# bao1029p/celestia-app

Measured on AMD Instinct MI355X. Metric: EDS+DAH squares/sec (128→256 sq, node) + RS GB/s & NMT SHA-256 hashes/sec, higher is better.
Workload: dtype u8; 1 GPU; 128x128 ODS -> 256x256 EDS + NMT row/col roots + DAH (configs[1]); k=128, global_batch=256, parallelism=squares sharded over 1 GPU(s), no collective, ods_layout=in place (Q0 of the EDS buffer)

## Files before the change

### celestia-app_amd/csrc/nmt.hip

```cpp
#include <hip/hip_runtime.h>
#include <stdint.h>
#include <stdlib.h>

#include "kernels.hpp"
#include "nmt_node.hpp"
#include "pipe_carve.hpp"
#include "sha256.hpp"

namespace dagpu {

constexpr int kLeafWave = 256;

__global__ __launch_bounds__(kLeafWave) void nmt_leaf_kernel(SquareArgs a, int row0, int nrows, int zero_status) {
  const int k = a.k;
  const long w = 2L * k;
  const long cells = w * w;
  const long span = nrows * w;
  const long total = span * a.nsq;
  const long gid = (long)blockIdx.x * kLeafWave + threadIdx.x;
  if (gid >= total) return;
  const long sq = gid / span;
  const long cell = row0 * w + (gid - sq * span);
  const long r = cell / w, c = cell - (cell / w) * w;
  const bool q0 = (r < k) && (c < k);
  if (zero_status && cell == 0) a.status[sq] = 0;
  const uint4* src = (const uint4*)(a.eds + sq * a.eds_sq_stride + cell * kShareSize);
  uint32_t st[8], ns[8];
  share_leaf_sha256(src, q0, st, ns);
  if (q0) {
    uint4* nsp = (uint4*)(a.ns_table + (sq * k * k + r * k + c) * 32);
    nsp[0] = make_uint4(ns[0], ns[1], ns[2], ns[3]);
    nsp[1] = make_uint4(ns[4], ns[5], ns[6], ns[7]);
  }
  uint4* out = (uint4*)(a.digests + (sq * cells + cell) * kDigest);
  out[0] = make_uint4(bswap32(st[0]), bswap32(st[1]), bswap32(st[2]), bswap32(st[3]));
  out[1] = make_uint4(bswap32(st[4]), bswap32(st[5]), bswap32(st[6]), bswap32(st[7]));
}

__device__ __forceinline__ void load_ns(const uint8_t* share, bool q0, uint32_t (&ns)[8]) {
  if (q0) {
    const uint4* p = (const uint4*)share;
    const uint4 v0 = p[0], v1 = p[1];
    ns[0] = v0.x; ns[1] = v0.y; ns[2] = v0.z; ns[3] = v0.w;
    ns[4] = v1.x; ns[5] = v1.y; ns[6] = v1.z; ns[7] = v1.w & 0xFFu;
  } else {
#pragma unroll
    for (int i = 0; i < 7; i++) ns[i] = 0xFFFFFFFFu;
    ns[7] = 0xFFu;
  }
}

constexpr uint32_t kParityRef = 0xFFFFFFFFu;

__device__ __forceinline__ void ns_by_ref(const uint8_t* ns_sq, uint32_t ref, uint32_t (&ns)[8]) {
  if (ref == kParityRef) {
#pragma unroll
    for (int i = 0; i < 7; i++) ns[i] = 0xFFFFFFFFu;
    ns[7] = 0xFFu;
  } else {
    const uint4* p = (const uint4*)(ns_sq + (long)ref * 32);
    const uint4 v0 = p[0], v1 = p[1];
    ns[0] = v0.x; ns[1] = v0.y; ns[2] = v0.z; ns[3] = v0.w;
    ns[4] = v1.x; ns[5] = v1.y; ns[6] = v1.z; ns[7] = v1.w;
  }
}

__device__ __forceinline__ void level_coords(long gid, int w, int per, long& sq, int& axis, int& idx, int& p) {
  const long blk = 2L * w * per;
  sq = gid / blk;
  const long g = gid - sq * blk;
  axis = g >= (long)w * per;
  const long g2 = g - (axis ? (long)w * per : 0);
  if (axis == 0) { idx = (int)(g2 / per); p = (int)(g2 - (long)idx * per); }
  else { p = (int)(g2 / w); idx = (int)(g2 - (long)p * w); }
}

__device__ __forceinline__ long level_rec(long sq, int w, int per, int axis, int idx, int p) {
  const long base = sq * 2L * w * per;
  return axis == 0 ? base + (long)idx * per + p : base + (long)w * per + (long)p * w + idx;
}

__global__ __launch_bounds__(256) void nmt_level1_kernel(SquareArgs a, uint8_t* out_rec, int final_level) {
  const int k = a.k;
  const int w = 2 * k;
  const int half = w / 2;
  const long gid = (long)blockIdx.x * 256 + threadIdx.x;
  const long total = a.nsq * 2L * w * half;
  if (gid >= total) return;
  long sq;
  int axis, idx, p;
  level_coords(gid, w, half, sq, axis, idx, p);
  const uint8_t* dig = a.digests + sq * (long)w * w * kDigest;
  const uint8_t* ns_sq = a.ns_table + sq * (long)k * k * 32;
  const int j0 = 2 * p, j1 = 2 * p + 1;
  const long cell0 = axis == 0 ? (long)idx * w + j0 : (long)j0 * w + idx;
  const long cell1 = axis == 0 ? (long)idx * w + j1 : (long)j1 * w + idx;
  const bool q00 = (idx < k) && (j0 < k), q01 = (idx < k) && (j1 < k);
  const uint32_t ref0 = q00 ? (axis == 0 ? (uint32_t)(idx * k + j0) : (uint32_t)(j0 * k + idx)) : kParityRef;
  const uint32_t ref1 = q01 ? (axis == 0 ? (uint32_t)(idx * k + j1) : (uint32_t)(j1 * k + idx)) : kParityRef;
  uint32_t nl[8], nr[8], dl[8], dr[8];
  ns_by_ref(ns_sq, ref0, nl);
  ns_by_ref(ns_sq, ref1, nr);
  load_digest(dig + cell0 * kDigest, dl);
  load_digest(dig + cell1 * kDigest, dr);
  if (q01) {
    bool bad = ns_less(nr, nl);
    if (j1 + 1 < k) {
      const uint32_t ref2 = axis == 0 ? (uint32_t)(idx * k + j1 + 1) : (uint32_t)((j1 + 1) * k + idx);
      uint32_t n2[8];
      ns_by_ref(ns_sq, ref2, n2);
      bad |= ns_less(n2, nr);
    }
    if (bad) atomicOr(&a.status[sq], kStatusPushOrder);
  }
  uint32_t st[8];
  const bool lpar = ns_is_parity(nl), rpar = ns_is_parity(nr);
  if (__all(lpar && rpar)) {
    auto get = [&](int P, int i) -> uint32_t {
      return P == 2 ? dl[i] : P == 5 ? dr[i] : 0xFFFFFFFFu;
    };
    sha_node_msg<true, true, true>(get, st);
  } else if (__all(lpar)) {
    auto get = [&](int P, int i) -> uint32_t {
      return P == 0 || P == 1 ? 0xFFFFFFFFu : P == 2 ? dl[i] : P == 3 || P == 4 ? nr[i] : dr[i];
    };
    sha_node_msg<true>(get, st);
  } else {
    auto get = [&](int P, int i) -> uint32_t {
      return P == 0 || P == 1 ? nl[i] : P == 2 ? dl[i] : P == 3 || P == 4 ? nr[i] : dr[i];
    };
    sha_node_msg(get, st);
  }
  uint32_t dg[8];
#pragma unroll
  for (int i = 0; i < 8; i++) dg[i] = bswap32(st[i]);
  if (final_level) {
    uint8_t* dst = (axis == 0 ? a.row_roots : a.col_roots) + (sq * w + idx) * kNodeSize;
    write_root(dst, nl, rpar ? nl : nr, dg);
  } else {
    const uint32_t lref = lpar ? kParityRef : ref0;
    const uint32_t rref = rpar ? kParityRef : ref1;
    uint4* o = (uint4*)(out_rec + gid * 48);
    o[0] = make_uint4(dg[0], dg[1], dg[2], dg[3]);
    o[1] = make_uint4(dg[4], dg[5], dg[6], dg[7]);
    o[2] = make_uint4(lref, rref == kParityRef ? lref : rref, 0u, 0u);
  }
}

__global__ __launch_bounds__(256) void nmt_level_kernel(SquareArgs a, const uint8_t* in_rec, uint8_t* out_rec,
                                                        int level, int final_level) {
  const int k = a.k;
  const int w = 2 * k;
  const int per = w >> level;
  const long gid = (long)blockIdx.x * 256 + threadIdx.x;
  const long total = a.nsq * 2L * w * per;
  if (gid >= total) return;
  long sq;
  int axis, idx, p;
  level_coords(gid, w, per, sq, axis, idx, p);
  const uint8_t* ns_sq = a.ns_table + sq * (long)k * k * 32;
  const uint4* li = (const uint4*)(in_rec + level_rec(sq, w, 2 * per, axis, idx, 2 * p) * 48);
  const uint4* ri = (const uint4*)(in_rec + level_rec(sq, w, 2 * per, axis, idx, 2 * p + 1) * 48);
  const uint4 l0 = li[0], l1 = li[1], l2 = li[2], r0 = ri[0], r1 = ri[1], r2 = ri[2];
  const uint32_t dl[8] = {l0.x, l0.y, l0.z, l0.w, l1.x, l1.y, l1.z, l1.w};
  const uint32_t dr[8] = {r0.x, r0.y, r0.z, r0.w, r1.x, r1.y, r1.z, r1.w};
  uint32_t lmn[8], lmx[8], rmn[8], rmx[8];
  ns_by_ref(ns_sq, l2.x, lmn);
  ns_by_ref(ns_sq, l2.y, lmx);
  ns_by_ref(ns_sq, r2.x, rmn);
  ns_by_ref(ns_sq, r2.y, rmx);
  uint32_t st[8];
  if (__all(l2.x == kParityRef && r2.x == kParityRef)) {
    auto get = [&](int P, int i) -> uint32_t {
      return P == 2 ? dl[i] : P == 5 ? dr[i] : 0xFFFFFFFFu;
    };
    sha_node_msg<true, true, true>(get, st);
  } else if (__all(l2.x == kParityRef)) {
    auto get = [&](int P, int i) -> uint32_t {
      return P <= 1 ? 0xFFFFFFFFu : P == 2 ? dl[i] : P == 3 ? rmn[i] : P == 4 ? rmx[i] : dr[i];
    };
    sha_node_msg<true>(get, st);
  } else {
    auto get = [&](int P, int i) -> uint32_t {
      return P == 0 ? lmn[i] : P == 1 ? lmx[i] : P == 2 ? dl[i] : P == 3 ? rmn[i] : P == 4 ? rmx[i] : dr[i];
    };
    sha_node_msg(get, st);
  }
  uint32_t dg[8];
#pragma unroll
  for (int i = 0; i < 8; i++) dg[i] = bswap32(st[i]);
  const bool rpar = r2.x == kParityRef;
  if (final_level) {
    uint8_t* dst = (axis == 0 ? a.row_roots : a.col_roots) + (sq * w + idx) * kNodeSize;
    if (rpar) write_root(dst, lmn, lmx, dg);
    else write_root(dst, lmn, rmx, dg);
  } else {
    uint4* o = (uint4*)(out_rec + gid * 48);
    o[0] = make_uint4(dg[0], dg[1], dg[2], dg[3]);
    o[1] = make_uint4(dg[4], dg[5], dg[6], dg[7]);
    o[2] = make_uint4(l2.x, rpar ? l2.y : r2.y, 0u, 0u);
  }
}

constexpr int kDahThreads = 1024;
constexpr int kDahChunk = 2048;

__device__ uint32_t* rfc_reduce(uint32_t* src, uint32_t* dst, int cur) {
  while (cur > 1) {
    const int next = cur / 2;
    for (int i = threadIdx.x; i < next; i += kDahThreads) {
      uint32_t m[32];
#pragma unroll
      for (int j = 0; j < 32; j++) m[j] = 0;
      uint32_t lft[8], rgt[8];
#pragma unroll
      for (int j = 0; j < 8; j++) { lft[j] = src[(2 * i) * 8 + j]; rgt[j] = src[(2 * i + 1) * 8 + j]; }
      m[0] = 0x01u;
      put_bytes<1>(m, lft);
      put_bytes<33>(m, rgt);
      m[65 >> 2] |= 0x80u << (8 * (65 & 3));
      uint32_t st[8];
      sha256_init(st);
#pragma unroll
      for (int blk = 0; blk < 2; blk++) {
        uint32_t wv[16];
#pragma unroll
        for (int j = 0; j < 16; j++) wv[j] = bswap32(m[16 * blk + j]);
        if (blk == 1) { wv[14] = 0; wv[15] = 65u * 8u; }
        sha256_compress(st, wv);
      }
#pragma unroll
      for (int j = 0; j < 8; j++) dst[i * 8 + j] = bswap32(st[j]);
    }
    __syncthreads();
    uint32_t* t = src;
    src = dst;
    dst = t;
    cur = next;
  }
  return src;
}

__device__ __forceinline__ void dah_leaf(const SquareArgs& a, long sq, int li, uint32_t* out) {
  const int w = 2 * a.k;
  const uint8_t* root = (li < w ? a.row_roots + (sq * w + li) * kNodeSize
                                : a.col_roots + (sq * w + (li - w)) * kNodeSize);
  uint32_t m[32];
#pragma unroll
  for (int j = 0; j < 32; j++) m[j] = 0;
  const uint16_t* r16 = (const uint16_t*)root;
#pragma unroll
  for (int h = 0; h < 45; h++) {
    const uint32_t v = r16[h];
    const int off = 1 + 2 * h;
    m[off >> 2] |= v << (8 * (off & 3));
    if ((off & 3) == 3) m[(off >> 2) + 1] |= v >> 8;
  }
  m[91 >> 2] |= 0x80u << (8 * (91 & 3));
  uint32_t st[8];
  sha256_init(st);
#pragma unroll
  for (int blk = 0; blk < 2; blk++) {
    uint32_t wv[16];
#pragma unroll
    for (int j = 0; j < 16; j++) wv[j] = bswap32(m[16 * blk + j]);
    if (blk == 1) { wv[14] = 0; wv[15] = 91u * 8u; }
    sha256_compress(st, wv);
  }
#pragma unroll
  for (int j = 0; j < 8; j++) out[j] = bswap32(st[j]);
}

__global__ __launch_bounds__(kDahThreads) void dah_kernel(SquareArgs a) {
  extern __shared__ __attribute__((aligned(16))) uint32_t lds[];
  const long sq = blockIdx.x;
  const int w = 2 * a.k;
  const int n = 2 * w;
  const int C = n < kDahChunk ? n : kDahChunk;
  uint32_t* sub = lds + (C + C / 2) * 8;
  for (int c0 = 0; c0 < n; c0 += C) {
    for (int i = threadIdx.x; i < C; i += kDahThreads) dah_leaf(a, sq, c0 + i, lds + i * 8);
    __syncthreads();
    const uint32_t* r = rfc_reduce(lds, lds + C * 8, C);
    if (threadIdx.x < 8) sub[(c0 / C) * 8 + threadIdx.x] = r[threadIdx.x];
    __syncthreads();
  }
  const uint32_t* root = rfc_reduce(sub, lds, n / C);
  if (threadIdx.x < 8) {
    uint32_t* out = (uint32_t*)(a.dah + sq * 32);
    out[threadIdx.x] = root[threadIdx.x];
  }
}

constexpr int kDahSub = 64;
__global__ __launch_bounds__(kDahSub) void dah_sub_kernel(SquareArgs a) {
  __shared__ __attribute__((aligned(16))) uint32_t buf[2][kDahSub * 8];
  const int n = 4 * a.k, per = n / kDahSub;
  const long sq = blockIdx.x / per;
  const int b = (int)(blockIdx.x % per);
  const int i = threadIdx.x;
  dah_leaf(a, sq, b * kDahSub + i, buf[0] + i * 8);
  int cur = kDahSub, src = 0;
  while (cur > 1) {
    __syncthreads();
    const int next = cur / 2;
    if (i < next) {
      uint32_t m[32];
#pragma unroll
      for (int j = 0; j < 32; j++) m[j] = 0;
      uint32_t lft[8], rgt[8];
#pragma unroll
      for (int j = 0; j < 8; j++) {
        lft[j] = buf[src][(2 * i) * 8 + j];
        rgt[j] = buf[src][(2 * i + 1) * 8 + j];
      }
      m[0] = 0x01u;
      put_bytes<1>(m, lft);
      put_bytes<33>(m, rgt);
      m[65 >> 2] |= 0x80u << (8 * (65 & 3));
      uint32_t st[8];
      sha256_init(st);
#pragma unroll
      for (int blk = 0; blk < 2; blk++) {
        uint32_t wv[16];
#pragma unroll
        for (int j = 0; j < 16; j++) wv[j] = bswap32(m[16 * blk + j]);
        if (blk == 1) { wv[14] = 0; wv[15] = 65u * 8u; }
        sha256_compress(st, wv);
      }
#pragma unroll
      for (int j = 0; j < 8; j++) buf[src ^ 1][i * 8 + j] = bswap32(st[j]);
    }
    src ^= 1;
    cur = next;
  }
  __syncthreads();
  if (i < 8) ((uint32_t*)a.digests)[blockIdx.x * 8 + i] = buf[src][i];
}

__global__ __launch_bounds__(kDahThreads) void dah_top_kernel(SquareArgs a) {
  extern __shared__ __attribute__((aligned(16))) uint32_t lds[];
  const long sq = blockIdx.x;
  const int per = 4 * a.k / kDahSub;
  const uint32_t* sub = (const uint32_t*)a.digests + sq * per * 8;
  for (int i = threadIdx.x; i < per * 8; i += kDahThreads) lds[i] = sub[i];
  __syncthreads();
  const uint32_t* root = rfc_reduce(lds, lds + per * 8, per);
  if (threadIdx.x < 8) ((uint32_t*)(a.dah + sq * 32))[threadIdx.x] = root[threadIdx.x];
}

hipError_t launch_nmt_leaves(const SquareArgs& a, hipStream_t s, int row0, int nrows, bool zero_status) {
  const long w = 2L * a.k;
  if (nrows < 0) nrows = (int)w - row0;
  if (row0 < 0 || nrows <= 0 || row0 + nrows > w || (zero_status && (row0 != 0 || !a.status)))
    return hipErrorInvalidValue;
  const long total = nrows * w * a.nsq;
  const long blocks = (total + kLeafWave - 1) / kLeafWave;
  hipLaunchKernelGGL(nmt_leaf_kernel, dim3((unsigned)blocks), dim3(kLeafWave), 0, s, a, row0, nrows,
                     (int)zero_status);
  return hipGetLastError();
}

hipError_t launch_nmt_tree_levels(const SquareArgs& a, int first, int last, uint8_t* const pp[2], uint8_t* last_out,
                                  hipStream_t s) {
  const int w = 2 * a.k;
  const int levels = nmt_levels(a.k);
  if (first < 1 || last > levels || first > last) return hipErrorInvalidValue;
  for (int L = first; L <= last; L++) {
    const uint8_t* in = pp[(L - first) & 1];
    uint8_t* out = L == last && last_out ? last_out : pp[(L - first + 1) & 1];
    const long total = a.nsq * 2L * w * (w >> L);
    const dim3 grid((unsigned)((total + 255) / 256));
    if (L == 1)
      hipLaunchKernelGGL(nmt_level1_kernel, grid, dim3(256), 0, s, a, out, (int)(levels == 1));
    else
      hipLaunchKernelGGL(nmt_level_kernel, grid, dim3(256), 0, s, a, in, out, L, (int)(L == levels));
    hipError_t e = hipGetLastError();
    if (e != hipSuccess) return e;
  }
  return hipSuccess;
}

hipError_t launch_nmt_trees(const SquareArgs& a, hipStream_t s) {
  uint8_t* const pp[2] = {a.rec_b, a.rec_a};
  return launch_nmt_tree_levels(a, 1, nmt_levels(a.k), pp, nullptr, s);
}

long nmt_level_fill_blocks() {
  static const long fill = [] {
    int dev = 0, cus = 0, per_cu = 0;
    if (hipGetDevice(&dev) != hipSuccess ||
        hipDeviceGetAttribute(&cus, hipDeviceAttributeMultiprocessorCount, dev) != hipSuccess ||
        hipOccupancyMaxActiveBlocksPerMultiprocessor(&per_cu, nmt_level_kernel, 256, 0) != hipSuccess ||
        cus <= 0 || per_cu <= 0) {
      (void)hipGetLastError();
      return 0L;
    }
    return (long)cus * per_cu;
  }();
  return fill;
}

size_t nmt_workspace_bytes(int k, long nsq) { return nmt_ws_bytes(k, nsq); }

void nmt_workspace_carve(SquareArgs& a, void* ws) {
  const NmtCarve c = nmt_carve(a.k, a.nsq);
  uint8_t* p = (uint8_t*)ws;
  a.digests = p + c.digests.off;
  a.ns_table = p + c.ns_table.off;
  a.rec_a = p + c.rec_a.off;
  a.rec_b = p + c.rec_b.off;
}

static bool dah_split_enabled() {
  const char* e = sw(SW_DAH_SPLIT);
  return !(e && e[0] == '0');
}

hipError_t launch_dah(const SquareArgs& a, hipStream_t s) {
  const int n = 4 * a.k;
  if (a.k > kMaxSplitK) return hipErrorInvalidValue;
  if (a.digests && n >= 1024 && a.nsq < 64 && dah_split_enabled()) {
    const int per = n / kDahSub;
    hipLaunchKernelGGL(dah_sub_kernel, dim3((unsigned)(a.nsq * per)), dim3(kDahSub), 0, s, a);
    hipError_t e = hipGetLastError();
    if (e != hipSuccess) return e;
    const size_t lds = (size_t)(per + per / 2) * 8 * sizeof(uint32_t);
    hipLaunchKernelGGL(dah_top_kernel, dim3((unsigned)a.nsq), dim3(kDahThreads), lds, s, a);
    return hipGetLastError();
  }
  const int C = n < kDahChunk ? n : kDahChunk;
  const size_t lds = ((size_t)(C + C / 2) + (size_t)(n / C)) * 8 * sizeof(uint32_t);
  if (lds > 65536) {
    hipError_t e = hipFuncSetAttribute((const void*)dah_kernel,
                                       hipFuncAttributeMaxDynamicSharedMemorySize, (int)lds);
    if (e != hipSuccess) return e;
  }
  hipLaunchKernelGGL(dah_kernel, dim3((unsigned)a.nsq), dim3(kDahThreads), lds, s, a);
  return hipGetLastError();
}

}
```

Measured before the change: 23280 squares/s.

## Specialize NMT kernels with power-of-two shift indexing and early parity exits

Templates the NMT leaf, level-1 and upper-level kernels on an index form. When sizes are powers of two, 64-bit divisions are replaced by 32-bit shifts and masks, with block-uniform square and axis decoding. The kernels also get launch_bounds occupancy hints and exit early on all-parity wavefronts, which skips namespace-table loads that are not needed. The cost is more template instantiations and register-pressure limits imposed by the min-waves hints, and non-power-of-two widths are now rejected in the tree-level path.

New measurement: 23450 squares/s, median of 6. Within noise of the previous version (+0.7%).

```diff
diff --git a/celestia-app_amd/csrc/nmt.hip b/celestia-app_amd/csrc/nmt.hip
--- a/celestia-app_amd/csrc/nmt.hip
+++ b/celestia-app_amd/csrc/nmt.hip
@@ -3,6 +3,7 @@
 #include <stdlib.h>
 
 #include "kernels.hpp"
+#include "nmt_index.hpp"
 #include "nmt_node.hpp"
 #include "pipe_carve.hpp"
 #include "sha256.hpp"
@@ -11,30 +12,65 @@
 
 constexpr int kLeafWave = 256;
 
-__global__ __launch_bounds__(kLeafWave) void nmt_leaf_kernel(SquareArgs a, int row0, int nrows, int zero_status) {
-  const int k = a.k;
-  const long w = 2L * k;
-  const long cells = w * w;
-  const long span = nrows * w;
-  const long total = span * a.nsq;
-  const long gid = (long)blockIdx.x * kLeafWave + threadIdx.x;
-  if (gid >= total) return;
-  const long sq = gid / span;
-  const long cell = row0 * w + (gid - sq * span);
-  const long r = cell / w, c = cell - (cell / w) * w;
-  const bool q0 = (r < k) && (c < k);
-  if (zero_status && cell == 0) a.status[sq] = 0;
-  const uint4* src = (const uint4*)(a.eds + sq * a.eds_sq_stride + cell * kShareSize);
+enum IndexForm { kIndexGeneric = 0, kIndexShift = 1, kIndexBlock = 2 };
+constexpr uint32_t kParityRef = 0xFFFFFFFFu;
+constexpr long kShiftLanes = 1L << 31;
+static inline bool is_pow2_l(long v) { return v > 0 && (v & (v - 1)) == 0; }
+static inline int log2_l(long v) { return __builtin_ctzl((unsigned long)v); }
+constexpr int leaf_waves(int form) { return form == kIndexGeneric ? 1 : 6; }
+constexpr int level1_waves(int form) { return form == kIndexGeneric ? 1 : 6; }
+constexpr int level_waves(int form) { return form == kIndexGeneric ? 1 : 5; }
+
+__device__ __forceinline__ void leaf_body(const uint8_t* src, bool q0, uint8_t* ns_sq, uint32_t ns_off,
+                                          uint8_t* out_p) {
   uint32_t st[8], ns[8];
-  share_leaf_sha256(src, q0, st, ns);
+  share_leaf_sha256((const uint4*)src, q0, st, ns);
   if (q0) {
-    uint4* nsp = (uint4*)(a.ns_table + (sq * k * k + r * k + c) * 32);
+    uint4* nsp = (uint4*)(ns_sq + ns_off);
     nsp[0] = make_uint4(ns[0], ns[1], ns[2], ns[3]);
     nsp[1] = make_uint4(ns[4], ns[5], ns[6], ns[7]);
   }
-  uint4* out = (uint4*)(a.digests + (sq * cells + cell) * kDigest);
+  uint4* out = (uint4*)out_p;
   out[0] = make_uint4(bswap32(st[0]), bswap32(st[1]), bswap32(st[2]), bswap32(st[3]));
   out[1] = make_uint4(bswap32(st[4]), bswap32(st[5]), bswap32(st[6]), bswap32(st[7]));
+}
+
+template <int FORM>
+__global__ __launch_bounds__(kLeafWave, leaf_waves(FORM)) void nmt_leaf_kernel(SquareArgs a, int row0, int nrows,
+                                                                                int zero_status, int lg_w,
+                                                                                int lg_span) {
+  const int k = a.k;
+  if constexpr (FORM == kIndexGeneric) {
+    const long w = 2L * k;
+    const long cells = w * w;
+    const long span = nrows * w;
+    const long total = span * a.nsq;
+    const long gid = (long)blockIdx.x * kLeafWave + threadIdx.x;
+    if (gid >= total) return;
+    const long sq = gid / span;
+    const long cell = row0 * w + (gid - sq * span);
+    const long r = cell / w, c = cell - (cell / w) * w;
+    const bool q0 = (r < k) && (c < k);
+    if (zero_status && cell == 0) a.status[sq] = 0;
+    leaf_body(a.eds + sq * a.eds_sq_stride + cell * kShareSize, q0, a.ns_table + sq * k * k * 32,
+              (uint32_t)((r * k + c) * 32), a.digests + (sq * cells + cell) * kDigest);
+  } else {
+    const uint32_t block0 = blockIdx.x * (uint32_t)kLeafWave;
+    const uint32_t lane = FORM == kIndexBlock ? threadIdx.x : 0u;
+    uint32_t sq, cell0;
+    const uint32_t first = block0 + (threadIdx.x - lane);
+    leaf_split(first, row0, lg_w, lg_span, sq, cell0);
+    if (FORM == kIndexShift ? first >= ((uint64_t)a.nsq << lg_span) : sq >= (uint64_t)a.nsq) return;
+    const uint32_t cell = cell0 + lane;
+    const uint32_t ref = cell_q0_ref(cell, lg_w, kParityRef);
+    const bool q0 = ref != kParityRef;
+    if (zero_status && cell == 0) a.status[sq] = 0;
+    const uint8_t* src = a.eds + (uint64_t)sq * (uint64_t)a.eds_sq_stride + ((uint64_t)cell0 << 9) + (lane << 9);
+    uint8_t* ns_sq = a.ns_table + ((uint64_t)sq << (2 * lg_w + 3));
+    uint8_t* out = a.digests + ((((uint64_t)sq << (2 * lg_w)) + cell0) << 5) + (lane << 5);
+    static_assert(kShareSize == 512 && kDigest == 32);
+    leaf_body(src, q0, ns_sq, ref << 5, out);
+  }
 }
 
 __device__ __forceinline__ void load_ns(const uint8_t* share, bool q0, uint32_t (&ns)[8]) {
@@ -50,7 +86,6 @@
   }
 }
 
-constexpr uint32_t kParityRef = 0xFFFFFFFFu;
 
 __device__ __forceinline__ void ns_by_ref(const uint8_t* ns_sq, uint32_t ref, uint32_t (&ns)[8]) {
   if (ref == kParityRef) {
@@ -58,12 +93,27 @@
     for (int i = 0; i < 7; i++) ns[i] = 0xFFFFFFFFu;
     ns[7] = 0xFFu;
   } else {
-    const uint4* p = (const uint4*)(ns_sq + (long)ref * 32);
+    const uint4* p = (const uint4*)(ns_sq + (ref << 5));
     const uint4 v0 = p[0], v1 = p[1];
     ns[0] = v0.x; ns[1] = v0.y; ns[2] = v0.z; ns[3] = v0.w;
     ns[4] = v1.x; ns[5] = v1.y; ns[6] = v1.z; ns[7] = v1.w;
   }
 }
+
+__device__ __forceinline__ void ns_parity(uint32_t (&ns)[8]) {
+#pragma unroll
+  for (int i = 0; i < 7; i++) ns[i] = 0xFFFFFFFFu;
+  ns[7] = 0xFFu;
+}
+
+struct LevelLane {
+  uint64_t sq;
+  uint32_t axis;
+  uint32_t tree;
+  uint32_t c0, c1;
+  const uint8_t *lp, *rp;
+  uint8_t* out;
+};
 
 __device__ __forceinline__ void level_coords(long gid, int w, int per, long& sq, int& axis, int& idx, int& p) {
   const long blk = 2L * w * per;
@@ -75,52 +125,110 @@
   else { p = (int)(g2 / w); idx = (int)(g2 - (long)p * w); }
 }
 
-__device__ __forceinline__ long level_rec(long sq, int w, int per, int axis, int idx, int p) {
-  const long base = sq * 2L * w * per;
-  return axis == 0 ? base + (long)idx * per + p : base + (long)w * per + (long)p * w + idx;
-}
-
-__global__ __launch_bounds__(256) void nmt_level1_kernel(SquareArgs a, uint8_t* out_rec, int final_level) {
-  const int k = a.k;
-  const int w = 2 * k;
-  const int half = w / 2;
-  const long gid = (long)blockIdx.x * 256 + threadIdx.x;
-  const long total = a.nsq * 2L * w * half;
-  if (gid >= total) return;
-  long sq;
-  int axis, idx, p;
-  level_coords(gid, w, half, sq, axis, idx, p);
-  const uint8_t* dig = a.digests + sq * (long)w * w * kDigest;
-  const uint8_t* ns_sq = a.ns_table + sq * (long)k * k * 32;
-  const int j0 = 2 * p, j1 = 2 * p + 1;
-  const long cell0 = axis == 0 ? (long)idx * w + j0 : (long)j0 * w + idx;
-  const long cell1 = axis == 0 ? (long)idx * w + j1 : (long)j1 * w + idx;
-  const bool q00 = (idx < k) && (j0 < k), q01 = (idx < k) && (j1 < k);
-  const uint32_t ref0 = q00 ? (axis == 0 ? (uint32_t)(idx * k + j0) : (uint32_t)(j0 * k + idx)) : kParityRef;
-  const uint32_t ref1 = q01 ? (axis == 0 ? (uint32_t)(idx * k + j1) : (uint32_t)(j1 * k + idx)) : kParityRef;
-  uint32_t nl[8], nr[8], dl[8], dr[8];
-  ns_by_ref(ns_sq, ref0, nl);
-  ns_by_ref(ns_sq, ref1, nr);
-  load_digest(dig + cell0 * kDigest, dl);
-  load_digest(dig + cell1 * kDigest, dr);
-  if (q01) {
-    bool bad = ns_less(nr, nl);
-    if (j1 + 1 < k) {
-      const uint32_t ref2 = axis == 0 ? (uint32_t)(idx * k + j1 + 1) : (uint32_t)((j1 + 1) * k + idx);
-      uint32_t n2[8];
-      ns_by_ref(ns_sq, ref2, n2);
-      bad |= ns_less(n2, nr);
-    }
-    if (bad) atomicOr(&a.status[sq], kStatusPushOrder);
-  }
-  uint32_t st[8];
-  const bool lpar = ns_is_parity(nl), rpar = ns_is_parity(nr);
-  if (__all(lpar && rpar)) {
+template <int FORM, int CHILD_STRIDE>
+__device__ __forceinline__ bool level_lane(const SquareArgs& a, const uint8_t* in, uint8_t* out_rec, int lg_w,
+                                           int lg_per, LevelLane& L) {
+  constexpr bool kLeaves = CHILD_STRIDE == kDigest;
+  const uint32_t tid = threadIdx.x;
+  const uint32_t w = 1u << lg_w;
+  if constexpr (FORM == kIndexGeneric) {
+    const int per = 1 << lg_per;
+    const long gid = (long)blockIdx.x * 256 + tid;
+    if (gid >= a.nsq * 2L * w * per) return false;
+    long sq;
+    int axis, idx, p;
+    level_coords(gid, (int)w, per, sq, axis, idx, p);
+    L.sq = (uint64_t)sq;
+    L.axis = (uint32_t)axis;
+    L.tree = (uint32_t)idx;
+    const uint64_t g2 = axis == 0 ? (uint64_t)idx * per + p : (uint64_t)p * w + idx;
+    L.c0 = (uint32_t)(axis == 0 ? 2 * g2 : g2 + (uint64_t)p * w);
+    L.c1 = L.c0 + (axis == 0 ? 1u : w);
+    const uint64_t sq_items = kLeaves ? (uint64_t)w * w : 4ull * w * per;
+    const uint64_t axis_items = kLeaves || axis == 0 ? 0 : 2ull * w * per;
+    L.lp = in + (L.sq * sq_items + axis_items + L.c0) * CHILD_STRIDE;
+    L.rp = in + (L.sq * sq_items + axis_items + L.c1) * CHILD_STRIDE;
+    L.out = out_rec + gid * 48;
+    return true;
+  } else {
+    const int lg_half = lg_w + lg_per;
+    const uint32_t block0 = blockIdx.x * 256u;
+    const uint32_t lane = FORM == kIndexBlock ? tid : 0u;
+    const uint32_t first = block0 + (tid - lane);
+    uint32_t sq, g0;
+    level_split(first, lg_half, sq, L.axis, g0);
+    if (FORM == kIndexShift ? first >= ((uint64_t)a.nsq << (lg_half + 1)) : sq >= (uint64_t)a.nsq) return false;
+    L.out = out_rec + (uint64_t)first * 48 + lane * 48u;
+    L.sq = sq;
+    const uint32_t g2 = g0 + lane;
+    L.tree = g2;
+    level_children(L.axis, g2, lg_w, L.c0, L.c1);
+    const uint64_t sq_axis = (kLeaves ? (uint64_t)sq : 2ull * sq + L.axis) << (lg_half + 1);
+    const uint8_t* base = in + sq_axis * CHILD_STRIDE;
+    if (L.axis == 0) {
+      L.lp = base + (uint64_t)g0 * (2 * CHILD_STRIDE) + lane * (2u * CHILD_STRIDE);
+      L.rp = L.lp + CHILD_STRIDE;
+    } else {
+      L.lp = base + (uint64_t)L.c0 * CHILD_STRIDE;
+      L.rp = L.lp + (w * (uint32_t)CHILD_STRIDE);
+    }
+    return true;
+  }
+}
+
+template <int FORM>
+__global__ __launch_bounds__(256, level1_waves(FORM)) void nmt_level1_kernel(SquareArgs a, uint8_t* out_rec,
+                                                                              int final_level, int lg_w) {
+  const uint32_t k = (uint32_t)a.k;
+  LevelLane L;
+  if (!level_lane<FORM, kDigest>(a, a.digests, out_rec, lg_w, lg_w - 1, L)) return;
+  const uint32_t ref0 = cell_q0_ref(L.c0, lg_w, kParityRef), ref1 = cell_q0_ref(L.c1, lg_w, kParityRef);
+  const bool q00 = ref0 != kParityRef, q01 = ref1 != kParityRef;
+  uint32_t dl[8], dr[8], st[8], dg[8];
+  load_digest(L.lp, dl);
+  load_digest(L.rp, dr);
+  auto root_dst = [&]() -> uint8_t* {
+    return (L.axis == 0 ? a.row_roots : a.col_roots) + ((L.sq << lg_w) + L.tree) * kNodeSize;
+  };
+  auto put_rec = [&](uint32_t mn, uint32_t mx) {
+    uint4* o = (uint4*)L.out;
+    o[0] = make_uint4(dg[0], dg[1], dg[2], dg[3]);
+    o[1] = make_uint4(dg[4], dg[5], dg[6], dg[7]);
+    o[2] = make_uint4(mn, mx, 0u, 0u);
+  };
+  if (__all(!q00)) {
     auto get = [&](int P, int i) -> uint32_t {
       return P == 2 ? dl[i] : P == 5 ? dr[i] : 0xFFFFFFFFu;
     };
     sha_node_msg<true, true, true>(get, st);
-  } else if (__all(lpar)) {
+#pragma unroll
+    for (int i = 0; i < 8; i++) dg[i] = bswap32(st[i]);
+    if (final_level) {
+      uint32_t np[8];
+      ns_parity(np);
+      write_root(root_dst(), np, np, dg);
+    } else {
+      put_rec(kParityRef, kParityRef);
+    }
+    return;
+  }
+  const uint8_t* ns_sq = a.ns_table + (L.sq << (2 * lg_w + 3));
+  uint32_t nl[8], nr[8];
+  ns_by_ref(ns_sq, ref0, nl);
+  ns_by_ref(ns_sq, ref1, nr);
+  if (q01) {
+    bool bad = ns_less(nr, nl);
+    const uint32_t j1 = L.axis == 0 ? L.c1 & ((1u << lg_w) - 1u) : L.c1 >> lg_w;
+    if (j1 + 1 < k) {
+      const uint32_t ref2 = ref1 + (L.axis == 0 ? 1u : k);
+      uint32_t n2[8];
+      ns_by_ref(ns_sq, ref2, n2);
+      bad |= ns_less(n2, nr);
+    }
+    if (bad) atomicOr(&a.status[L.sq], kStatusPushOrder);
+  }
+  const bool lpar = ns_is_parity(nl), rpar = ns_is_parity(nr);
+  if (__all(lpar)) {
     auto get = [&](int P, int i) -> uint32_t {
       return P == 0 || P == 1 ? 0xFFFFFFFFu : P == 2 ? dl[i] : P == 3 || P == 4 ? nr[i] : dr[i];
     };
@@ -131,75 +239,87 @@
     };
     sha_node_msg(get, st);
   }
-  uint32_t dg[8];
 #pragma unroll
   for (int i = 0; i < 8; i++) dg[i] = bswap32(st[i]);
   if (final_level) {
-    uint8_t* dst = (axis == 0 ? a.row_roots : a.col_roots) + (sq * w + idx) * kNodeSize;
-    write_root(dst, nl, rpar ? nl : nr, dg);
+    write_root(root_dst(), nl, rpar ? nl : nr, dg);
   } else {
     const uint32_t lref = lpar ? kParityRef : ref0;
     const uint32_t rref = rpar ? kParityRef : ref1;
-    uint4* o = (uint4*)(out_rec + gid * 48);
-    o[0] = make_uint4(dg[0], dg[1], dg[2], dg[3]);
-    o[1] = make_uint4(dg[4], dg[5], dg[6], dg[7]);
-    o[2] = make_uint4(lref, rref == kParityRef ? lref : rref, 0u, 0u);
-  }
-}
-
-__global__ __launch_bounds__(256) void nmt_level_kernel(SquareArgs a, const uint8_t* in_rec, uint8_t* out_rec,
-                                                        int level, int final_level) {
-  const int k = a.k;
-  const int w = 2 * k;
-  const int per = w >> level;
-  const long gid = (long)blockIdx.x * 256 + threadIdx.x;
-  const long total = a.nsq * 2L * w * per;
-  if (gid >= total) return;
-  long sq;
-  int axis, idx, p;
-  level_coords(gid, w, per, sq, axis, idx, p);
-  const uint8_t* ns_sq = a.ns_table + sq * (long)k * k * 32;
-  const uint4* li = (const uint4*)(in_rec + level_rec(sq, w, 2 * per, axis, idx, 2 * p) * 48);
-  const uint4* ri = (const uint4*)(in_rec + level_rec(sq, w, 2 * per, axis, idx, 2 * p + 1) * 48);
+    put_rec(lref, rref == kParityRef ? lref : rref);
+  }
+}
+
+template <int FORM>
+__global__ __launch_bounds__(256, level_waves(FORM)) void nmt_level_kernel(SquareArgs a, const uint8_t* in_rec,
+                                                                            uint8_t* out_rec, int level,
+                                                                            int final_level, int lg_w) {
+  LevelLane L;
+  if (!level_lane<FORM, 48>(a, in_rec, out_rec, lg_w, lg_w - level, L)) return;
+  const uint4 *li = (const uint4*)L.lp, *ri = (const uint4*)L.rp;
   const uint4 l0 = li[0], l1 = li[1], l2 = li[2], r0 = ri[0], r1 = ri[1], r2 = ri[2];
   const uint32_t dl[8] = {l0.x, l0.y, l0.z, l0.w, l1.x, l1.y, l1.z, l1.w};
   const uint32_t dr[8] = {r0.x, r0.y, r0.z, r0.w, r1.x, r1.y, r1.z, r1.w};
-  uint32_t lmn[8], lmx[8], rmn[8], rmx[8];
-  ns_by_ref(ns_sq, l2.x, lmn);
-  ns_by_ref(ns_sq, l2.y, lmx);
-  ns_by_ref(ns_sq, r2.x, rmn);
-  ns_by_ref(ns_sq, r2.y, rmx);
-  uint32_t st[8];
-  if (__all(l2.x == kParityRef && r2.x == kParityRef)) {
+  const bool rpar = r2.x == kParityRef;
+  const uint8_t* ns_sq = a.ns_table + (L.sq << (2 * lg_w + 3));
+  uint32_t st[8], dg[8];
+  auto put = [&](const uint32_t (&mn)[8], const uint32_t (&mx)[8]) {
+#pragma unroll
+    for (int i = 0; i < 8; i++) dg[i] = bswap32(st[i]);
+    if (final_level) {
+      uint8_t* dst = (L.axis == 0 ? a.row_roots : a.col_roots) + ((L.sq << lg_w) + L.tree) * kNodeSize;
+      write_root(dst, mn, mx, dg);
+    } else {
+      uint4* o = (uint4*)L.out;
+      o[0] = make_uint4(dg[0], dg[1], dg[2], dg[3]);
+      o[1] = make_uint4(dg[4], dg[5], dg[6], dg[7]);
+      o[2] = make_uint4(l2.x, rpar ? l2.y : r2.y, 0u, 0u);
+    }
+  };
+  if (__all(l2.x == kParityRef && rpar)) {
     auto get = [&](int P, int i) -> uint32_t {
       return P == 2 ? dl[i] : P == 5 ? dr[i] : 0xFFFFFFFFu;
     };
     sha_node_msg<true, true, true>(get, st);
-  } else if (__all(l2.x == kParityRef)) {
+    uint32_t np[8];
+    ns_parity(np);
+    if (final_level) {
+      uint32_t lmx[8];
+      ns_by_ref(ns_sq, l2.y, lmx);
+      put(np, lmx);
+    } else {
+      put(np, np);
+    }
+    return;
+  }
+  uint32_t rmn[8], rmx[8];
+  ns_by_ref(ns_sq, r2.x, rmn);
+  ns_by_ref(ns_sq, r2.y, rmx);
+  if (__all(l2.x == kParityRef)) {
     auto get = [&](int P, int i) -> uint32_t {
       return P <= 1 ? 0xFFFFFFFFu : P == 2 ? dl[i] : P == 3 ? rmn[i] : P == 4 ? rmx[i] : dr[i];
     };
     sha_node_msg<true>(get, st);
-  } else {
-    auto get = [&](int P, int i) -> uint32_t {
-      return P == 0 ? lmn[i] : P == 1 ? lmx[i] : P == 2 ? dl[i] : P == 3 ? rmn[i] : P == 4 ? rmx[i] : dr[i];
-    };
-    sha_node_msg(get, st);
-  }
-  uint32_t dg[8];
-#pragma unroll
-  for (int i = 0; i < 8; i++) dg[i] = bswap32(st[i]);
-  const bool rpar = r2.x == kParityRef;
-  if (final_level) {
-    uint8_t* dst = (axis == 0 ? a.row_roots : a.col_roots) + (sq * w + idx) * kNodeSize;
-    if (rpar) write_root(dst, lmn, lmx, dg);
-    else write_root(dst, lmn, rmx, dg);
-  } else {
-    uint4* o = (uint4*)(out_rec + gid * 48);
-    o[0] = make_uint4(dg[0], dg[1], dg[2], dg[3]);
-    o[1] = make_uint4(dg[4], dg[5], dg[6], dg[7]);
-    o[2] = make_uint4(l2.x, rpar ? l2.y : r2.y, 0u, 0u);
-  }
+    uint32_t np[8];
+    ns_parity(np);
+    if (rpar) {
+      uint32_t lmx[8];
+      ns_by_ref(ns_sq, l2.y, lmx);
+      put(np, lmx);
+    } else {
+      put(np, rmx);
+    }
+    return;
+  }
+  uint32_t lmn[8], lmx[8];
+  ns_by_ref(ns_sq, l2.x, lmn);
+  ns_by_ref(ns_sq, l2.y, lmx);
+  auto get = [&](int P, int i) -> uint32_t {
+    return P == 0 ? lmn[i] : P == 1 ? lmx[i] : P == 2 ? dl[i] : P == 3 ? rmn[i] : P == 4 ? rmx[i] : dr[i];
+  };
+  sha_node_msg(get, st);
+  if (rpar) put(lmn, lmx);
+  else put(lmn, rmx);
 }
 
 constexpr int kDahThreads = 1024;
@@ -354,10 +474,19 @@
   if (nrows < 0) nrows = (int)w - row0;
   if (row0 < 0 || nrows <= 0 || row0 + nrows > w || (zero_status && (row0 != 0 || !a.status)))
     return hipErrorInvalidValue;
-  const long total = nrows * w * a.nsq;
-  const long blocks = (total + kLeafWave - 1) / kLeafWave;
-  hipLaunchKernelGGL(nmt_leaf_kernel, dim3((unsigned)blocks), dim3(kLeafWave), 0, s, a, row0, nrows,
-                     (int)zero_status);
+  const long span = nrows * w;
+  const long total = span * a.nsq;
+  const dim3 grid((unsigned)((total + kLeafWave - 1) / kLeafWave)), block(kLeafWave);
+  const bool shifts = is_pow2_l(w) && is_pow2_l(span) && total < kShiftLanes;
+  const int lg_w = shifts ? log2_l(w) : 0, lg_span = shifts ? log2_l(span) : 0;
+  if (!shifts)
+    hipLaunchKernelGGL(nmt_leaf_kernel<kIndexGeneric>, grid, block, 0, s, a, row0, nrows, (int)zero_status, 0, 0);
+  else if (span >= kLeafWave)
+    hipLaunchKernelGGL(nmt_leaf_kernel<kIndexBlock>, grid, block, 0, s, a, row0, nrows, (int)zero_status, lg_w,
+                       lg_span);
+  else
+    hipLaunchKernelGGL(nmt_leaf_kernel<kIndexShift>, grid, block, 0, s, a, row0, nrows, (int)zero_status, lg_w,
+                       lg_span);
   return hipGetLastError();
 }
 
@@ -365,16 +494,31 @@
                                   hipStream_t s) {
   const int w = 2 * a.k;
   const int levels = nmt_levels(a.k);
-  if (first < 1 || last > levels || first > last) return hipErrorInvalidValue;
+  if (first < 1 || last > levels || first > last || !is_pow2_l(w)) return hipErrorInvalidValue;
+  const int lg_w = log2_l(w);
   for (int L = first; L <= last; L++) {
     const uint8_t* in = pp[(L - first) & 1];
     uint8_t* out = L == last && last_out ? last_out : pp[(L - first + 1) & 1];
-    const long total = a.nsq * 2L * w * (w >> L);
-    const dim3 grid((unsigned)((total + 255) / 256));
-    if (L == 1)
-      hipLaunchKernelGGL(nmt_level1_kernel, grid, dim3(256), 0, s, a, out, (int)(levels == 1));
-    else
-      hipLaunchKernelGGL(nmt_level_kernel, grid, dim3(256), 0, s, a, in, out, L, (int)(L == levels));
+    const long axis_nodes = (long)w * (w >> L);
+    const long total = a.nsq * 2L * axis_nodes;
+    const dim3 grid((unsigned)((total + 255) / 256)), block(256);
+    const int form = total >= kShiftLanes ? kIndexGeneric : axis_nodes >= 256 ? kIndexBlock : kIndexShift;
+    const int fin = (int)(L == levels);
+    if (L == 1) {
+      if (form == kIndexBlock)
+        hipLaunchKernelGGL(nmt_level1_kernel<kIndexBlock>, grid, block, 0, s, a, out, fin, lg_w);
+      else if (form == kIndexShift)
+        hipLaunchKernelGGL(nmt_level1_kernel<kIndexShift>, grid, block, 0, s, a, out, fin, lg_w);
+      else
+        hipLaunchKernelGGL(nmt_level1_kernel<kIndexGeneric>, grid, block, 0, s, a, out, fin, lg_w);
+    } else {
+      if (form == kIndexBlock)
+        hipLaunchKernelGGL(nmt_level_kernel<kIndexBlock>, grid, block, 0, s, a, in, out, L, fin, lg_w);
+      else if (form == kIndexShift)
+        hipLaunchKernelGGL(nmt_level_kernel<kIndexShift>, grid, block, 0, s, a, in, out, L, fin, lg_w);
+      else
+        hipLaunchKernelGGL(nmt_level_kernel<kIndexGeneric>, grid, block, 0, s, a, in, out, L, fin, lg_w);
+    }
     hipError_t e = hipGetLastError();
     if (e != hipSuccess) return e;
   }
@@ -391,7 +535,7 @@
     int dev = 0, cus = 0, per_cu = 0;
     if (hipGetDevice(&dev) != hipSuccess ||
         hipDeviceGetAttribute(&cus, hipDeviceAttributeMultiprocessorCount, dev) != hipSuccess ||
-        hipOccupancyMaxActiveBlocksPerMultiprocessor(&per_cu, nmt_level_kernel, 256, 0) != hipSuccess ||
+        hipOccupancyMaxActiveBlocksPerMultiprocessor(&per_cu, nmt_level_kernel<kIndexBlock>, 256, 0) != hipSuccess ||
         cus <= 0 || per_cu <= 0) {
       (void)hipGetLastError();
       return 0L;
diff --git a/celestia-app_amd/csrc/nmt_index.hpp b/celestia-app_amd/csrc/nmt_index.hpp
--- /dev/null
+++ b/celestia-app_amd/csrc/nmt_index.hpp
@@ -0,0 +1,34 @@
+#pragma once
+#include <stdint.h>
+
+#if defined(__HIPCC__)
+#define DAGPU_IDX_HD __host__ __device__ __forceinline__
+#else
+#define DAGPU_IDX_HD inline
+#endif
+
+namespace dagpu {
+
+DAGPU_IDX_HD void leaf_split(uint32_t first, int row0, int lg_w, int lg_span, uint32_t& sq, uint32_t& cell0) {
+  sq = first >> lg_span;
+  cell0 = ((uint32_t)row0 << lg_w) + (first & ((1u << lg_span) - 1u));
+}
+
+DAGPU_IDX_HD void level_split(uint32_t first, int lg_half, uint32_t& sq, uint32_t& axis, uint32_t& g0) {
+  sq = first >> (lg_half + 1);
+  axis = (first >> lg_half) & 1u;
+  g0 = first & ((1u << lg_half) - 1u);
+}
+
+DAGPU_IDX_HD void level_children(uint32_t axis, uint32_t g2, int lg_w, uint32_t& c0, uint32_t& c1) {
+  const uint32_t w = 1u << lg_w;
+  c0 = axis == 0 ? 2u * g2 : g2 + (g2 & ~(w - 1u));
+  c1 = c0 + (axis == 0 ? 1u : w);
+}
+
+DAGPU_IDX_HD uint32_t cell_q0_ref(uint32_t cell, int lg_w, uint32_t none) {
+  const uint32_t k = 1u << (lg_w - 1), r = cell >> lg_w, c = cell & ((2u * k) - 1u);
+  return r < k && c < k ? (r << (lg_w - 1)) + c : none;
+}
+
+}
```
